# Seba-san/icm-slam

Hardware: NVIDIA B200
Metric: ICM sweeps/sec (1M poses,100k lmk) at 1/2/4/8 B200; % HBM roofline (higher is better)
Workload: dtype f64

## Files before the change

### icm_slam_b200/csrc/solve.cuh

```cuda
#pragma once
#include "common.cuh"

#define ST_SLOTS 64
#define ST_THREADS ST_SLOTS
#define ST_OWN (2 * ST_SLOTS - 2)
#define ST_XT (2 * ST_SLOTS + 4)
#define ST_MINB 8

__global__ void k_odo_increments(const double* __restrict__ odo, int64_t ldo, int T, double* __restrict__ inc, int64_t ldi)
{
    int t = blockIdx.x * blockDim.x + threadIdx.x;
    if (t >= T) return;
    double dx = 0.0, dy = 0.0, dth = 0.0;
    if (t + 1 < T) {
        double s, c;
        sincos(odo[2 * ldo + t], &s, &c);
        const double vx = odo[t + 1] - odo[t], vy = odo[ldo + t + 1] - odo[ldo + t];
        dx = c * vx + s * vy;
        dy = -s * vx + c * vy;
        dth = odo[2 * ldo + t + 1] - odo[2 * ldo + t];
    }
    inc[t] = dx; inc[ldi + t] = dy; inc[2 * ldi + t] = dth;
}

__global__ void __launch_bounds__(128)
k_body_moments(const int* __restrict__ off, const double2* __restrict__ bxy, int T, double* __restrict__ bm, int64_t ld)
{
    const int t = blockIdx.x * blockDim.x + threadIdx.x;
    if (t >= T) return;
    double Bx = 0.0, By = 0.0, Bxx = 0.0, Byy = 0.0, Bxy = 0.0;
    for (int i = off[t]; i < off[t + 1]; ++i) {
        const double2 b = bxy[i];
        Bx += b.x; By += b.y;
        Bxx = fma(b.x, b.x, Bxx); Byy = fma(b.y, b.y, Byy); Bxy = fma(b.x, b.y, Bxy);
    }
    bm[t] = Bx; bm[ld + t] = By; bm[2 * ld + t] = Bxx; bm[3 * ld + t] = Byy; bm[4 * ld + t] = Bxy;
    bm[5 * ld + t] = (double)(off[t + 1] - off[t]);
}

__global__ void k_interleave(const double* __restrict__ bx, const double* __restrict__ by, int64_t n, double2* __restrict__ out)
{
    const int64_t i = (int64_t)blockIdx.x * blockDim.x + threadIdx.x;
    if (i < n) out[i] = make_double2(bx[i], by[i]);
}

struct TrajLayout {
    int first;
    int traj_T;
    const double* x0s;
    int64_t ldx0s;
    double x0[3];
    __device__ __forceinline__ bool pinned(int t) const { return traj_T > 0 ? (t % traj_T) == 0 : (t == 0 && first); }
    __device__ __forceinline__ bool after_pinned(int t) const { return traj_T > 0 ? (t % traj_T) == 1 : (t == 1 && first); }
    __device__ __forceinline__ bool has_next(int t, int T) const { return t + 1 < T && (traj_T == 0 || ((t + 1) % traj_T) != 0); }
    __device__ __forceinline__ double x0_of(int t, int r) const { return traj_T > 0 ? x0s[r * ldx0s + t / traj_T] : x0[r]; }
};

__global__ void k_ppar_init(const double* __restrict__ x, int64_t ld, int t_begin, int t_end, const TrajLayout L, double4* __restrict__ ppar)
{
    const int t = t_begin + blockIdx.x * blockDim.x + threadIdx.x;
    if (t >= t_end) return;
    if (L.pinned(t)) ppar[t] = make_ppar(L.x0_of(t, 0), L.x0_of(t, 1), L.x0_of(t, 2));
    else ppar[t] = make_ppar(x[t], x[ld + t], x[2 * ld + t]);
}

__device__ __forceinline__ double entrepi_fast(double a)
{
    return (fabs(a) <= ICM_PI) ? a : entrepi(a);
}

__device__ __forceinline__ void sincos_small(double d, double& s, double& c)
{
    const double z = d * d;
    s = d * fma(z, fma(z, fma(z, fma(z, fma(z, -2.5052108385441719e-08, 2.7557319223985893e-06), -1.9841269841269841e-04),
                              8.3333333333333332e-03), -1.6666666666666666e-01), 1.0);
    c = fma(z, fma(z, fma(z, fma(z, fma(z, -2.7557319223985888e-07, 2.4801587301587302e-05), -1.3888888888888889e-03),
                          4.1666666666666664e-02), -0.5), 1.0);
}

struct Mom {
    double n, Bx, By, Bxx, Byy, Bxy, Yx, Yy, Mxx, Mxy, Myx, Myy;
};

struct PoseIn {
    double ax, ay, ath, sa, ca;
    double bx, by, bth;
    double uav, uaw, ucv, ucw;
    double D0x, D0y, dth0;
    double D1x, D1y, dth1;
    int has_next;
};

struct RowCoef {
    double iS, KA, P1, P2;
    double ba, bb, bab, bd;
};

__device__ __forceinline__ RowCoef row_coef(const Mom& M, double r, double q, double k, double dt, double hn, double dv, double D1x,
                                            double D1y, double kD1x, double kD1y, double uav, double a_, double hu, double e0i,
                                            double bp, double Y, double M1, double M2)
{
    RowCoef R;
    const double ga = fma(mul_rn(hu, uav), dt, a_);
    const double e0 = add_rn(a_, e0i);
    const double rk = add_rn(r, k), rdv = mul_rn(r, dv);
    R.iS = 1.0 / fma(hn, rk, fma(M.n, q, rk));
    R.KA = fma(rk, bp, fma(q, Y, fma(ga, r, mul_rn(k, e0))));
    R.P1 = fma(q, M.By, add_rn(rdv, kD1x));
    R.P2 = fma(q, M.Bx, -kD1y);
    const double iKA = mul_rn(R.iS, R.KA);
    R.ba = fma(iKA, R.P2, fma(mul_rn(k, bp), D1y, -mul_rn(q, M1)));
    R.bb = fma(-iKA, R.P1, fma(bp, fma(r, dv, kD1x), mul_rn(q, M2)));
    R.bab = fma(-R.iS, fma(R.P2, R.P2, -mul_rn(R.P1, R.P1)),
                fma(q, sub_rn(M.Bxx, M.Byy), -fma(rdv, dv, mul_rn(k, fma(D1x, D1x, -mul_rn(D1y, D1y))))));
    R.bd = fma(-mul_rn(R.iS, R.P1), R.P2, fma(q, M.Bxy, -mul_rn(kD1x, D1y)));
    return R;
}

__device__ __forceinline__ int newton_trig(const DevCfg& cfg, const PoseIn& P, const Mom& M, double ox, double oy, double& th,
                                           double s, double c, double tol, int maxit, double& x, double& y)
{
    const double dt = cfg.dt, k = cfg.kod;
    const double hn = P.has_next ? 1.0 : 0.0;
    const double D1x = mul_rn(hn, P.D1x), D1y = mul_rn(hn, P.D1y);
    const double dv = mul_rn(mul_rn(hn, dt), P.ucv);
    const double kD1x = mul_rn(k, D1x), kD1y = mul_rn(k, D1y);
    const RowCoef X = row_coef(M, cfg.r1, cfg.q1, k, dt, hn, dv, D1x, D1y, kD1x, kD1y, P.uav, sub_rn(P.ax, ox), P.ca,
                               fma(P.ca, P.D0x, -mul_rn(P.sa, P.D0y)), mul_rn(hn, sub_rn(P.bx, ox)), M.Yx, M.Mxx, M.Mxy);
    const RowCoef Y = row_coef(M, cfg.r2, cfg.q2, k, dt, hn, dv, D1x, D1y, kD1x, kD1y, P.uav, sub_rn(P.ay, oy), P.sa,
                               fma(P.ca, P.D0y, mul_rn(P.sa, P.D0x)), mul_rn(hn, sub_rn(P.by, oy)), M.Yy, M.Myx, M.Myy);
    const double as2 = 2.0 * add_rn(X.bb, Y.ba), ac2 = 2.0 * sub_rn(X.ba, Y.bb);
    const double au2 = 2.0 * sub_rn(X.bab, Y.bab), av2 = 2.0 * sub_rn(X.bd, Y.bd);
    const double av8 = 4.0 * av2;
    const double ang2 = (2.0 * cfg.r3 + 2.0 * k) * (1.0 + hn);
    const double r3_2 = 2.0 * cfg.r3, k_2 = 2.0 * k;
    const double th_ga = fma(dt, P.uaw, P.ath), c3 = add_rn(P.dth0, P.ath), c4 = sub_rn(P.dth1, P.bth), wb = fma(dt, P.ucw, -P.bth);
    int it = 0;
    bool done = false;
    for (;;) {
        const double u = s * c, v = fma(c, c, -s * s);
        double ang1 = fma(r3_2, entrepi_fast(th - th_ga), -k_2 * entrepi_fast(c3 - th));
        if (P.has_next) ang1 += fma(r3_2, entrepi_fast(th + wb), k_2 * entrepi_fast(c4 + th));
        const double p1 = fma(as2, s, fma(ac2, c, fma(au2, u, fma(av2, v, ang1))));
        double p2 = fma(as2, c, fma(-ac2, s, fma(au2, v, fma(-av8, u, ang2))));
        if (!(p2 > 0.0)) p2 = ang2;
        const double dth = mul_rn(-p1, (double)__frcp_rn((float)p2));
        if (!done) {
            th = add_rn(th, dth);
            ++it;
            if (fabs(dth) <= 0.125) {
                double sd, cd;
                sincos_small(dth, sd, cd);
                const double s2 = fma(s, cd, c * sd);
                c = fma(c, cd, -s * sd);
                s = s2;
            } else {
                sincos(th, &s, &c);
            }
            done = fabs(dth) <= tol || it >= maxit;
        }
        if (__all_sync(FULLMASK, done)) break;
    }
    x = fma(fma(-s, X.P2, fma(-c, X.P1, X.KA)), X.iS, ox);
    y = fma(fma(c, Y.P2, fma(-s, Y.P1, Y.KA)), Y.iS, oy);
    return it;
}

struct SolveParams {
    int T;
    int t_lo, t_hi;
    TrajLayout lay;
    const double* xin; int64_t ldin;
    double* xout; int64_t ldout;
    const double* inc; int64_t ldinc;
    const double* u; int64_t ldu;
    const double* bm; int64_t ldbm;
    const double* dyn;
    const double4* ppin; double4* ppout;
    DevCfg cfg;
    double tol; int maxit;
    unsigned long long* iters;
    int tile0;
    unsigned long long* trace_row;
    const unsigned* trace_seq;
    Freeze fz;
};

struct __align__(16) SolveSmem {
    double xs[3][ST_XT];
    double xn[3][ST_XT];
    double inc[3][ST_XT];
    double u[2][ST_XT];
    double sn[ST_XT], cs[ST_XT];
};

struct SlotMom {
    Mom M;
    bool valid, pinned;
    int t, li;
};

template <bool FZ>
__device__ __forceinline__ SlotMom solve_slot_load(const SolveParams& p, int tb, int q, int phase)
{
    SlotMom s;
    s.t = phase == 0 ? tb - 1 + 2 * q : tb + 2 * q;
    s.li = s.t - (tb - 2);
    s.valid = s.t >= 0 && s.t < p.t_hi && (phase == 0 ? (q == 0 || s.t >= p.t_lo) : (q != ST_SLOTS - 1 && s.t >= p.t_lo));
    s.pinned = s.valid && (p.lay.pinned(s.t) || (FZ && p.fz.scan(s.t)));
    Mom& M = s.M;
    M.n = M.Bx = M.By = M.Bxx = M.Byy = M.Bxy = M.Yx = M.Yy = M.Mxx = M.Mxy = M.Myx = M.Myy = 0.0;
    if (s.valid && !s.pinned) {
        const double* bmq = p.bm + s.t;
        M.n = __ldg(bmq + 5 * p.ldbm);
        M.Bx = __ldg(bmq); M.By = __ldg(bmq + p.ldbm); M.Bxx = __ldg(bmq + 2 * p.ldbm);
        M.Byy = __ldg(bmq + 3 * p.ldbm); M.Bxy = __ldg(bmq + 4 * p.ldbm);
        const double2* d = reinterpret_cast<const double2*>(p.dyn + (size_t)s.t * 6);
        const double2 d0 = d[0], d1 = d[1], d2 = d[2];
        M.Yx = d0.x; M.Mxx = d0.y; M.Mxy = d1.x; M.Yy = d1.y; M.Myx = d2.x; M.Myy = d2.y;
    }
    return s;
}

template <bool FZ>
__global__ void __launch_bounds__(ST_THREADS, ST_MINB)
k_solve_tile(const SolveParams p)
{
    __shared__ SolveSmem S;
    const int q = threadIdx.x;
    if (p.trace_row && blockIdx.x == 0 && q == 0) { unsigned long long t; asm volatile("mov.u64 %0, %%globaltimer;" : "=l"(t)); p.trace_row[((*p.trace_seq) & 31) * 8 + 5] = t; }
    const int tb = p.t_lo + (p.tile0 + blockIdx.x) * ST_OWN;
    const int T = p.T;
    SlotMom cur = solve_slot_load<FZ>(p, tb, q, 0);
    for (int li = q; li < ST_XT; li += ST_THREADS) {
        const int t = tb - 2 + li;
        const bool ok = t >= 0 && t < T;
        double th = 0.0;
        for (int r = 0; r < 3; ++r) {
            const double v = ok ? p.xin[r * p.ldin + t] : 0.0;
            S.xs[r][li] = v; S.xn[r][li] = v;
            S.inc[r][li] = ok ? p.inc[r * p.ldinc + t] : 0.0;
            if (r == 2) th = v;
        }
        S.u[0][li] = ok ? p.u[t] : 0.0;
        S.u[1][li] = ok ? p.u[p.ldu + t] : 0.0;
        double sh = 0.0, ch = 1.0;
        if (ok) {
            if (p.lay.pinned(t)) sincos(th, &sh, &ch);
            else { const double4 pq = ldg_ppar(p.ppin + t); sh = pq.w; ch = -pq.z; }
        }
        S.sn[li] = sh; S.cs[li] = ch;
    }
    __syncthreads();
    int my_iters = 0;
    for (int phase = 0; phase < 2; ++phase) {
        const Mom& M = cur.M;
        const int t = cur.t, li = cur.li;
        const bool qvalid = cur.valid, pinned = cur.pinned;
        double rx = 0.0, ry = 0.0, th = 0.0;
        PoseIn P;
        P.ax = P.ay = P.ath = P.sa = 0.0; P.ca = 1.0; P.bx = P.by = P.bth = 0.0; P.uav = P.uaw = P.ucv = P.ucw = 0.0;
        P.D0x = P.D0y = P.dth0 = P.D1x = P.D1y = P.dth1 = 0.0; P.has_next = 0;
        bool solve = false;
        double ox = 0.0, oy = 0.0, th0 = 0.0, s0 = 0.0, c0 = 1.0;
        if (qvalid) {
            double (*X)[ST_XT] = phase == 0 ? S.xs : S.xn;
            const bool has_next = p.lay.has_next(t, T);
            solve = !pinned && M.n > 0.0;
            ox = S.xs[0][li]; oy = S.xs[1][li]; th0 = S.xs[2][li]; s0 = S.sn[li]; c0 = S.cs[li];
            th = th0;
            if (!pinned) {
                P.ax = X[0][li - 1]; P.ay = X[1][li - 1]; P.ath = X[2][li - 1];
                P.sa = S.sn[li - 1]; P.ca = S.cs[li - 1];
                if (has_next) { P.bx = X[0][li + 1]; P.by = X[1][li + 1]; P.bth = X[2][li + 1]; }
                P.uav = S.u[0][li - 1]; P.uaw = S.u[1][li - 1];
                P.ucv = S.u[0][li]; P.ucw = S.u[1][li];
                P.D0x = S.inc[0][li - 1]; P.D0y = S.inc[1][li - 1]; P.dth0 = S.inc[2][li - 1];
                P.D1x = S.inc[0][li]; P.D1y = S.inc[1][li]; P.dth1 = S.inc[2][li];
                P.has_next = has_next ? 1 : 0;
                if (!solve) {
                    const bool t1 = p.lay.after_pinned(t);
                    rx = ((t1 ? p.lay.x0_of(t - 1, 0) : X[0][li - 1]) + X[0][li + 1]) / 2.0;
                    ry = ((t1 ? p.lay.x0_of(t - 1, 1) : X[1][li - 1]) + X[1][li + 1]) / 2.0;
                    th = ((t1 ? p.lay.x0_of(t - 1, 2) : X[2][li - 1]) + X[2][li + 1]) / 2.0;
                }
            }
        }
        {
            double x2 = 0.0, y2 = 0.0, th2 = th0;
            const int it = newton_trig(p.cfg, P, M, ox, oy, th2, s0, c0, p.tol, solve ? p.maxit : 1, x2, y2);
            if (solve) { rx = x2; ry = y2; th = th2; my_iters += it; }
        }
        SlotMom nxt = cur;
        if (phase == 0) nxt = solve_slot_load<FZ>(p, tb, q, 1);
        if (qvalid && !pinned) {
            double st, ct;
            sincos(sub_rn(th, ICM_HALFPI), &st, &ct);
            S.xn[0][li] = rx; S.xn[1][li] = ry; S.xn[2][li] = th;
            S.sn[li] = ct; S.cs[li] = -st;
        }
        __syncthreads();
        cur = nxt;
    }
    if (p.iters) {
        my_iters = warp_sum_i(my_iters);
        if ((q & 31) == 0 && my_iters) atomicAdd(p.iters, (unsigned long long)my_iters);
    }
    const int n_own = min(ST_OWN, p.t_hi - tb);
    for (int r = 0; r < 3; ++r)
        for (int k = q; k < n_own; k += ST_THREADS) p.xout[r * p.ldout + tb + k] = S.xn[r][k + 2];
    for (int k = q; k < n_own; k += ST_THREADS) {
        const int tt = tb + k, l2 = k + 2;
        if (p.lay.pinned(tt)) p.ppout[tt] = make_ppar(p.lay.x0_of(tt, 0), p.lay.x0_of(tt, 1), p.lay.x0_of(tt, 2));
        else if (FZ && p.fz.scan(tt)) p.ppout[tt] = ldg_ppar(p.ppin + tt);
        else p.ppout[tt] = make_double4(S.xn[0][l2], S.xn[1][l2], -S.cs[l2], S.sn[l2]);
    }
}
```

Before: 4822.

## Park Newton row coefficients in shared memory to cut register pressure

Moves the per-row back-substitution coefficients (inverse, KA, P1, P2) into a shared-memory park area during the Newton loop and reloads them afterward. The next phase's slot moments are now loaded only at the start of phase 1 instead of being prefetched, and the non-solve midpoint fallback is deferred past the solve. Together with raising min blocks per SM from 8 to 10, this aims to lower live registers so more blocks fit per SM. It costs extra shared memory per block and some shared loads and stores, and gives up the overlap from the earlier prefetch.

```diff
diff --git a/icm_slam_b200/csrc/solve.cuh b/icm_slam_b200/csrc/solve.cuh
--- a/icm_slam_b200/csrc/solve.cuh
+++ b/icm_slam_b200/csrc/solve.cuh
@@ -5,7 +5,7 @@
 #define ST_THREADS ST_SLOTS
 #define ST_OWN (2 * ST_SLOTS - 2)
 #define ST_XT (2 * ST_SLOTS + 4)
-#define ST_MINB 8
+#define ST_MINB 10
 
 __global__ void k_odo_increments(const double* __restrict__ odo, int64_t ldo, int T, double* __restrict__ inc, int64_t ldi)
 {
@@ -92,49 +92,58 @@
 };
 
 struct RowCoef {
-    double iS, KA, P1, P2;
+    double KA, P1, P2;
     double ba, bb, bab, bd;
 };
 
-__device__ __forceinline__ RowCoef row_coef(const Mom& M, double r, double q, double k, double dt, double hn, double dv, double D1x,
-                                            double D1y, double kD1x, double kD1y, double uav, double a_, double hu, double e0i,
-                                            double bp, double Y, double M1, double M2)
+__device__ __forceinline__ double row_inv(const Mom& M, double r, double q, double k, double hn)
+{
+    const double rk = add_rn(r, k);
+    return 1.0 / fma(hn, rk, fma(M.n, q, rk));
+}
+
+__device__ __forceinline__ RowCoef row_coef(const Mom& M, double iS, double r, double q, double k, double dt, double hn, double dv,
+                                            double D1x, double D1y, double kD1x, double kD1y, double uav, double a_, double hu,
+                                            double e0i, double bp, double Y, double M1, double M2)
 {
     RowCoef R;
     const double ga = fma(mul_rn(hu, uav), dt, a_);
     const double e0 = add_rn(a_, e0i);
     const double rk = add_rn(r, k), rdv = mul_rn(r, dv);
-    R.iS = 1.0 / fma(hn, rk, fma(M.n, q, rk));
     R.KA = fma(rk, bp, fma(q, Y, fma(ga, r, mul_rn(k, e0))));
     R.P1 = fma(q, M.By, add_rn(rdv, kD1x));
     R.P2 = fma(q, M.Bx, -kD1y);
-    const double iKA = mul_rn(R.iS, R.KA);
+    const double iKA = mul_rn(iS, R.KA);
     R.ba = fma(iKA, R.P2, fma(mul_rn(k, bp), D1y, -mul_rn(q, M1)));
     R.bb = fma(-iKA, R.P1, fma(bp, fma(r, dv, kD1x), mul_rn(q, M2)));
-    R.bab = fma(-R.iS, fma(R.P2, R.P2, -mul_rn(R.P1, R.P1)),
+    R.bab = fma(-iS, fma(R.P2, R.P2, -mul_rn(R.P1, R.P1)),
                 fma(q, sub_rn(M.Bxx, M.Byy), -fma(rdv, dv, mul_rn(k, fma(D1x, D1x, -mul_rn(D1y, D1y))))));
-    R.bd = fma(-mul_rn(R.iS, R.P1), R.P2, fma(q, M.Bxy, -mul_rn(kD1x, D1y)));
+    R.bd = fma(-mul_rn(iS, R.P1), R.P2, fma(q, M.Bxy, -mul_rn(kD1x, D1y)));
     return R;
 }
 
-__device__ __forceinline__ int newton_trig(const DevCfg& cfg, const PoseIn& P, const Mom& M, double ox, double oy, double& th,
-                                           double s, double c, double tol, int maxit, double& x, double& y)
-{
+__device__ __forceinline__ int newton_trig(const DevCfg& cfg, const PoseIn& P, const Mom& M, const double* o, double* park,
+                                           double& th, double s, double c, double tol, int maxit, double& x, double& y)
+{
+    const double ox = o[0], oy = o[ST_XT];
     const double dt = cfg.dt, k = cfg.kod;
     const double hn = P.has_next ? 1.0 : 0.0;
+    const double th_ga = fma(dt, P.uaw, P.ath), c3 = add_rn(P.dth0, P.ath), c4 = sub_rn(P.dth1, P.bth), wb = fma(dt, P.ucw, -P.bth);
     const double D1x = mul_rn(hn, P.D1x), D1y = mul_rn(hn, P.D1y);
     const double dv = mul_rn(mul_rn(hn, dt), P.ucv);
     const double kD1x = mul_rn(k, D1x), kD1y = mul_rn(k, D1y);
-    const RowCoef X = row_coef(M, cfg.r1, cfg.q1, k, dt, hn, dv, D1x, D1y, kD1x, kD1y, P.uav, sub_rn(P.ax, ox), P.ca,
+    const double iSx = row_inv(M, cfg.r1, cfg.q1, k, hn), iSy = row_inv(M, cfg.r2, cfg.q2, k, hn);
+    const RowCoef X = row_coef(M, iSx, cfg.r1, cfg.q1, k, dt, hn, dv, D1x, D1y, kD1x, kD1y, P.uav, sub_rn(P.ax, ox), P.ca,
                                fma(P.ca, P.D0x, -mul_rn(P.sa, P.D0y)), mul_rn(hn, sub_rn(P.bx, ox)), M.Yx, M.Mxx, M.Mxy);
-    const RowCoef Y = row_coef(M, cfg.r2, cfg.q2, k, dt, hn, dv, D1x, D1y, kD1x, kD1y, P.uav, sub_rn(P.ay, oy), P.sa,
+    const RowCoef Y = row_coef(M, iSy, cfg.r2, cfg.q2, k, dt, hn, dv, D1x, D1y, kD1x, kD1y, P.uav, sub_rn(P.ay, oy), P.sa,
                                fma(P.ca, P.D0y, mul_rn(P.sa, P.D0x)), mul_rn(hn, sub_rn(P.by, oy)), M.Yy, M.Myx, M.Myy);
+    park[0 * ST_THREADS] = iSx; park[1 * ST_THREADS] = X.KA; park[2 * ST_THREADS] = X.P1; park[3 * ST_THREADS] = X.P2;
+    park[4 * ST_THREADS] = iSy; park[5 * ST_THREADS] = Y.KA; park[6 * ST_THREADS] = Y.P1; park[7 * ST_THREADS] = Y.P2;
     const double as2 = 2.0 * add_rn(X.bb, Y.ba), ac2 = 2.0 * sub_rn(X.ba, Y.bb);
     const double au2 = 2.0 * sub_rn(X.bab, Y.bab), av2 = 2.0 * sub_rn(X.bd, Y.bd);
     const double av8 = 4.0 * av2;
     const double ang2 = (2.0 * cfg.r3 + 2.0 * k) * (1.0 + hn);
     const double r3_2 = 2.0 * cfg.r3, k_2 = 2.0 * k;
-    const double th_ga = fma(dt, P.uaw, P.ath), c3 = add_rn(P.dth0, P.ath), c4 = sub_rn(P.dth1, P.bth), wb = fma(dt, P.ucw, -P.bth);
     int it = 0;
     bool done = false;
     for (;;) {
@@ -161,8 +170,9 @@
         }
         if (__all_sync(FULLMASK, done)) break;
     }
-    x = fma(fma(-s, X.P2, fma(-c, X.P1, X.KA)), X.iS, ox);
-    y = fma(fma(c, Y.P2, fma(-s, Y.P1, Y.KA)), Y.iS, oy);
+    asm volatile("" ::: "memory");
+    x = fma(fma(-s, park[3 * ST_THREADS], fma(-c, park[2 * ST_THREADS], park[1 * ST_THREADS])), park[0], o[0]);
+    y = fma(fma(c, park[7 * ST_THREADS], fma(-s, park[6 * ST_THREADS], park[5 * ST_THREADS])), park[4 * ST_THREADS], o[ST_XT]);
     return it;
 }
 
@@ -192,6 +202,7 @@
     double inc[3][ST_XT];
     double u[2][ST_XT];
     double sn[ST_XT], cs[ST_XT];
+    double park[8][ST_THREADS];
 };
 
 struct SlotMom {
@@ -252,23 +263,21 @@
         S.sn[li] = sh; S.cs[li] = ch;
     }
     __syncthreads();
-    int my_iters = 0;
     for (int phase = 0; phase < 2; ++phase) {
+        if (phase == 1) cur = solve_slot_load<FZ>(p, tb, q, 1);
         const Mom& M = cur.M;
         const int t = cur.t, li = cur.li;
         const bool qvalid = cur.valid, pinned = cur.pinned;
-        double rx = 0.0, ry = 0.0, th = 0.0;
+        double (*X)[ST_XT] = phase == 0 ? S.xs : S.xn;
         PoseIn P;
         P.ax = P.ay = P.ath = P.sa = 0.0; P.ca = 1.0; P.bx = P.by = P.bth = 0.0; P.uav = P.uaw = P.ucv = P.ucw = 0.0;
         P.D0x = P.D0y = P.dth0 = P.D1x = P.D1y = P.dth1 = 0.0; P.has_next = 0;
         bool solve = false;
-        double ox = 0.0, oy = 0.0, th0 = 0.0, s0 = 0.0, c0 = 1.0;
+        double th0 = 0.0, s0 = 0.0, c0 = 1.0;
         if (qvalid) {
-            double (*X)[ST_XT] = phase == 0 ? S.xs : S.xn;
             const bool has_next = p.lay.has_next(t, T);
             solve = !pinned && M.n > 0.0;
-            ox = S.xs[0][li]; oy = S.xs[1][li]; th0 = S.xs[2][li]; s0 = S.sn[li]; c0 = S.cs[li];
-            th = th0;
+            th0 = S.xs[2][li]; s0 = S.sn[li]; c0 = S.cs[li];
             if (!pinned) {
                 P.ax = X[0][li - 1]; P.ay = X[1][li - 1]; P.ath = X[2][li - 1];
                 P.sa = S.sn[li - 1]; P.ca = S.cs[li - 1];
@@ -278,33 +287,32 @@
                 P.D0x = S.inc[0][li - 1]; P.D0y = S.inc[1][li - 1]; P.dth0 = S.inc[2][li - 1];
                 P.D1x = S.inc[0][li]; P.D1y = S.inc[1][li]; P.dth1 = S.inc[2][li];
                 P.has_next = has_next ? 1 : 0;
-                if (!solve) {
-                    const bool t1 = p.lay.after_pinned(t);
-                    rx = ((t1 ? p.lay.x0_of(t - 1, 0) : X[0][li - 1]) + X[0][li + 1]) / 2.0;
-                    ry = ((t1 ? p.lay.x0_of(t - 1, 1) : X[1][li - 1]) + X[1][li + 1]) / 2.0;
-                    th = ((t1 ? p.lay.x0_of(t - 1, 2) : X[2][li - 1]) + X[2][li + 1]) / 2.0;
-                }
             }
         }
+        double rx = 0.0, ry = 0.0, th = th0;
         {
             double x2 = 0.0, y2 = 0.0, th2 = th0;
-            const int it = newton_trig(p.cfg, P, M, ox, oy, th2, s0, c0, p.tol, solve ? p.maxit : 1, x2, y2);
-            if (solve) { rx = x2; ry = y2; th = th2; my_iters += it; }
-        }
-        SlotMom nxt = cur;
-        if (phase == 0) nxt = solve_slot_load<FZ>(p, tb, q, 1);
+            const int it = newton_trig(p.cfg, P, M, &S.xs[0][li], &S.park[0][q], th2, s0, c0, p.tol, solve ? p.maxit : 1, x2,
+                                       y2);
+            if (solve) { rx = x2; ry = y2; th = th2; }
+            if (p.iters) {
+                const int w = warp_sum_i(solve ? it : 0);
+                if ((q & 31) == 0 && w) atomicAdd(p.iters, (unsigned long long)w);
+            }
+        }
         if (qvalid && !pinned) {
+            if (!solve) {
+                const bool t1 = p.lay.after_pinned(t);
+                rx = ((t1 ? p.lay.x0_of(t - 1, 0) : X[0][li - 1]) + X[0][li + 1]) / 2.0;
+                ry = ((t1 ? p.lay.x0_of(t - 1, 1) : X[1][li - 1]) + X[1][li + 1]) / 2.0;
+                th = ((t1 ? p.lay.x0_of(t - 1, 2) : X[2][li - 1]) + X[2][li + 1]) / 2.0;
+            }
             double st, ct;
             sincos(sub_rn(th, ICM_HALFPI), &st, &ct);
             S.xn[0][li] = rx; S.xn[1][li] = ry; S.xn[2][li] = th;
             S.sn[li] = ct; S.cs[li] = -st;
         }
         __syncthreads();
-        cur = nxt;
-    }
-    if (p.iters) {
-        my_iters = warp_sum_i(my_iters);
-        if ((q & 31) == 0 && my_iters) atomicAdd(p.iters, (unsigned long long)my_iters);
     }
     const int n_own = min(ST_OWN, p.t_hi - tb);
     for (int r = 0; r < 3; ++r)
```

Measured after the change: 4901 (median of 6 runs). 1.02x the previous value.
